# cvlab-stonybrook/s-volsdf

Measured on AMD Instinct MI355X. Metric: rendered rays/sec (1024-ray batch, 128 samples), higher is better.
Workload: dtype f32 (every product, forward and backward, as three fp16 MFMA products of two-piece fp16 operands with f32 accumulate; activation blocks hold both pieces: float32 accuracy class); 1 GPU; configs[1]: VolOpt.train_step (forward + MVS prior lookup + loss + backward + clip/guard/Adam), train mode, fast=1: 1024 rays/GPU x 128 coarse + 98 composited samples + 2048 eikonal points, 8x256 SDF MLP + 4x256 radiance MLP; mode=train, mlp_precision=fp16x2, launch=eager launches, rays_per_gpu=1024, rays_total=1024

## Files before the change

### s-volsdf_amd/csrc/svs_wgrad.hip

```cpp
#include "svs_common.h"
#include "svs_mlp_layout.h"
#include "svs_ticket.h"
#include <cstdlib>

namespace svs {
namespace wgrad {

struct Pair {
  const float* a;
  const float* b;
  size_t stride_a, stride_b;
};

struct Args {
  Pair p[2];
  int n_pairs;
  int n_tiles;
  int n_valid_points;
  const float* b_extra;
  size_t stride_extra;
  float* dW;
  int ldw;
  float* db;
  det::Ticket ticket;
};

struct Staging {
  f32x4 a[8], b[8], x;
};

template <int NTB>
__global__ __launch_bounds__(256, 1) void wgrad_kernel(Args a) {
  constexpr int PA = 260, PB = NTB == 9 ? 292 : 260;
  constexpr int BUF = 32 * (PA + PB);
  extern __shared__ __attribute__((aligned(16))) float smem[];
  const int tid = threadIdx.x, wave = tid >> 6, lane = tid & 63;
  const int half = lane >> 5, col = lane & 31;
  f32x16 acc[2][NTB];
#pragma unroll
  for (int o = 0; o < 2; ++o)
#pragma unroll
    for (int i = 0; i < NTB; ++i) acc[o][i] = (f32x16)(0.0f);
  float bias_acc = 0.0f;

  const int my_tiles = a.n_tiles > (int)blockIdx.x ? (a.n_tiles - 1 - (int)blockIdx.x) / (int)gridDim.x + 1 : 0;
  const int n_items = my_tiles * a.n_pairs;
  Staging st;
  int st_live = 32;

  auto issue = [&](int item) {
    const int t = blockIdx.x + (item / a.n_pairs) * gridDim.x, pi = item % a.n_pairs;
    const Pair& p = a.p[pi];
    const f32x4* ga = reinterpret_cast<const f32x4*>(p.a + (size_t)t * p.stride_a);
    const f32x4* gb = reinterpret_cast<const f32x4*>(p.b + (size_t)t * p.stride_b);
#pragma unroll
    for (int k = 0; k < 8; ++k) { st.a[k] = ga[k * 256 + tid]; st.b[k] = gb[k * 256 + tid]; }
    if (NTB == 9) {
      st.x = (a.b_extra && pi == 0) ? reinterpret_cast<const f32x4*>(a.b_extra + (size_t)t * a.stride_extra)[tid]
                                    : (f32x4)(0.0f);
    }
    st_live = a.n_valid_points - t * 32;
  };
  auto commit = [&](int buf) {
    float* la = smem + buf * BUF;
    float* lb = la + 32 * PA;
    if (st_live < 32) {
#pragma unroll
      for (int k = 0; k < 8; ++k) if ((tid & 31) >= st_live) st.a[k] = (f32x4)(0.0f);
    }
#pragma unroll
    for (int k = 0; k < 8; ++k) {
      const int q = k * 256 + tid, i4 = q >> 6, ln = q & 63;
      const int feat = 32 * (i4 >> 2) + 8 * (i4 & 3) + 4 * (ln >> 5), pt = ln & 31;
      *reinterpret_cast<f32x4*>(la + pt * PA + feat) = st.a[k];
      *reinterpret_cast<f32x4*>(lb + pt * PB + feat) = st.b[k];
    }
    if (NTB == 9) {
      const int i4 = tid >> 6, ln = tid & 63;
      *reinterpret_cast<f32x4*>(lb + (ln & 31) * PB + 256 + 8 * i4 + 4 * (ln >> 5)) = st.x;
    }
  };

  if (n_items > 0) { issue(0); commit(0); }
  __syncthreads();
  for (int item = 0; item < n_items; ++item) {
    const int buf = item & 1;
    const bool more = item + 1 < n_items;
    if (more) issue(item + 1);
    const float* la = smem + buf * BUF;
    const float* lb = la + 32 * PA;
    if (a.db && (item % a.n_pairs) == 0) {
      float s = 0.0f;
#pragma unroll 8
      for (int q = 0; q < 32; ++q) s += la[q * PA + tid];
      bias_acc += s;
    }
#pragma unroll 4
    for (int s = 0; s < 16; ++s) {
      const int pt = 2 * s + half;
      const float a0 = la[pt * PA + 32 * (2 * wave) + col];
      const float a1 = la[pt * PA + 32 * (2 * wave + 1) + col];
#pragma unroll
      for (int i = 0; i < NTB; ++i) {
        const float b = lb[pt * PB + 32 * i + col];
        acc[0][i] = __builtin_amdgcn_mfma_f32_32x32x2f32(a0, b, acc[0][i], 0, 0, 0);
        acc[1][i] = __builtin_amdgcn_mfma_f32_32x32x2f32(a1, b, acc[1][i], 0, 0, 0);
      }
    }
    if (more) commit(buf ^ 1);
    __syncthreads();
  }
  det::wait_turn(a.ticket, blockIdx.x);
#pragma unroll
  for (int o = 0; o < 2; ++o)
#pragma unroll
    for (int i = 0; i < NTB; ++i)
#pragma unroll
      for (int r = 0; r < 16; ++r) {
        const int row = 32 * (2 * wave + o) + rho(r) + 4 * half;
        const int c = 32 * i + col;
        if (c < a.ldw) atomicAdd(&a.dW[(size_t)row * a.ldw + c], acc[o][i][r]);
      }
  if (a.db) atomicAdd(&a.db[tid], bias_acc);
  det::pass_turn(a.ticket, blockIdx.x);
}


namespace h2 {

typedef _Float16 f16x8 __attribute__((ext_vector_type(8)));
typedef _Float16 f16x4 __attribute__((ext_vector_type(4)));
typedef _Float16 f16x2 __attribute__((ext_vector_type(2)));
typedef short s16x4 __attribute__((__vector_size__(4 * sizeof(short))));
#define SVS_LDS(T, ptr) ((__attribute__((address_space(3))) T*)(ptr))

constexpr int kPlane = 16384;
constexpr int kExtraPiece = 32 * 64;
constexpr int kNarrowImg = 8192;
constexpr int kRecBytes = 8 * 256;
constexpr int kFactorBytes = 8 * 64;
template <bool GP>
struct Ring {
  static constexpr int kPlanes = GP ? 2 : 1;
  static constexpr int kSlot = 2 * kPlanes * kPlane;
  static constexpr int kB = kPlanes * kPlane;
  static constexpr int kRing = GP ? 2 : 4;
  static constexpr int kAhead = kRing - 1;
  static constexpr int kSlotAll = kSlot + kRecBytes + kFactorBytes;
  static constexpr int kLdsBytes = kRing * kSlotAll;
};

struct Frag { s16x4 lo, hi; };
__device__ __forceinline__ void tr_issue(Frag& v, unsigned a0, unsigned a1) {
  asm volatile("ds_read_b64_tr_b16 %0, %1" : "=v"(v.lo) : "v"(a0));
  asm volatile("ds_read_b64_tr_b16 %0, %1" : "=v"(v.hi) : "v"(a1));
}
__device__ __forceinline__ f16x8 frag_of(const Frag& v) { return __builtin_bit_cast(f16x8, v); }
__device__ __forceinline__ void lds_read128(f32x4& v, unsigned a) { asm volatile("ds_read_b128 %0, %1" : "=v"(v) : "v"(a)); }
__device__ __forceinline__ void lds_read32(float& v, unsigned a) { asm volatile("ds_read_b32 %0, %1" : "=v"(v) : "v"(a)); }
__device__ __forceinline__ void lds_wait() {
  asm volatile("s_waitcnt lgkmcnt(0)" ::: "memory");
  __builtin_amdgcn_sched_barrier(0);
}
__device__ __forceinline__ unsigned lds_addr(const void* p) {
  return (unsigned)(unsigned long long)SVS_LDS(const void, p);
}

__device__ __forceinline__ void scale_from_absmax(const float* absmax, float& s, float& inv_s) {
  s = 1.0f; inv_s = 1.0f;
  if (!absmax) return;
  int e = (int)((__float_as_uint(*absmax) >> 23) & 0xff);
  e = e < 16 ? 16 : (e > 250 ? 250 : e);
  s = __uint_as_float((unsigned)(268 - e) << 23);
  inv_s = __uint_as_float((unsigned)(e - 14) << 23);
}

struct Job {
  Pair p[2];
  const float* rec[2];
  int n_pairs;
  int n_tiles;
  int n_valid_points;
  int b_tiles;
  int col0;
  float* dW;
  int ldw;
  float* db;
  const float* absmax;
  int wg_begin, wg_count;
  det::Ticket ticket;
};
constexpr int kMaxJobs = 20;
struct MultiArgs { Job job[kMaxJobs]; int n_jobs; int touch; int reverse; };
static_assert(sizeof(MultiArgs) <= 4096, "kernel arguments");

constexpr int kThreadsW = 512;

typedef const __attribute__((address_space(1))) void* gvoid;

template <bool GP>
__global__ __launch_bounds__(kThreadsW, 1) void wgrad_h2_multi_kernel(MultiArgs ma) {
  typedef Ring<GP> R;
  constexpr int kSlot = R::kSlot, kSlotAll = R::kSlotAll, kRing = R::kRing, kAhead = R::kAhead, kB = R::kB;
  extern __shared__ __attribute__((aligned(16))) unsigned char smem_h2[];
  int jj = 0;
  for (int q = 1; q < ma.n_jobs; ++q) if ((int)blockIdx.x >= ma.job[q].wg_begin) jj = q;
  const Job& a = ma.job[jj];
  const int wg = (int)blockIdx.x - a.wg_begin, nwg = a.wg_count;
  const int tid = threadIdx.x, lane = tid & 63;
  const int wave = __builtin_amdgcn_readfirstlane(tid >> 6);
  const bool narrow = a.b_tiles == 1;
  float s_grad, inv_s;
  scale_from_absmax(a.absmax, s_grad, inv_s);

  f32x16 acc[8];
#pragma unroll
  for (int i = 0; i < 8; ++i) acc[i] = (f32x16)(0.0f);
  float bsum = 0.0f;

  unsigned char* ring = smem_h2;

  const int rq = (lane & 15) >> 2, rp = lane & 3, rg = (lane >> 4) & 1, rh = lane >> 5;
  const int rd0 = 1024 * rg + 256 * rh + 128 * rg + 64 * (rp & 1) + 16 * rq + 8 * (rp >> 1);
  const int a_rd = 2048 * wave + rd0;
  const int rx0 = 64 * (8 * rh + rq) + 32 * rg + 8 * rp, rx1 = rx0 + 64 * 4;
  const int wp = lane & 31, whf = lane >> 5;
  const int wxoff = 64 * wp + 16 * (wave & 3) + 8 * whf;

  const bool two_pairs = a.n_pairs == 2;
  const int my_tiles = a.n_tiles > wg ? (a.n_tiles - 1 - wg) / nwg + 1 : 0;
  const int n_items = two_pairs ? 2 * my_tiles : my_tiles;
  const int n_valid = a.n_valid_points;
  const bool has_db = a.db != nullptr;
  const bool rev = ma.reverse != 0;
  const float* const pa0 = a.p[0].a; const float* const pb0 = a.p[0].b;
  const float* const pa1 = a.p[1].a; const float* const pb1 = a.p[1].b;
  const size_t sa0 = a.p[0].stride_a, sb0 = a.p[0].stride_b, sa1 = a.p[1].stride_a, sb1 = a.p[1].stride_b;
  const float* const rec0 = a.rec[0]; const float* const rec1 = a.rec[1];
  const bool has_scale = a.absmax != nullptr;
  auto tile_of = [&](int item) {
    const int k = two_pairs ? item >> 1 : item;
    return rev ? wg + (my_tiles - 1 - k) * nwg : wg + k * nwg;
  };

  auto issue = [&](int item) {
    const int t = tile_of(item), pi = two_pairs ? item & 1 : 0;
    const float* pa = (pi ? pa1 : pa0) + (size_t)t * (pi ? sa1 : sa0);
    const float* pb = (pi ? pb1 : pb0) + (size_t)t * (pi ? sb1 : sb0);
    unsigned char* slot = ring + (item % kRing) * kSlotAll;
#pragma unroll
    for (int j = 0; j < 2 * R::kPlanes; ++j) {
      const int piece = wave + 8 * j;
      __builtin_amdgcn_global_load_lds((gvoid)(reinterpret_cast<const f32x4*>(pa) + piece * 64 + lane),
                                       SVS_LDS(void, slot + piece * 1024), 16, 0, 0);
      if (!narrow)
        __builtin_amdgcn_global_load_lds((gvoid)(reinterpret_cast<const f32x4*>(pb) + piece * 64 + lane),
                                         SVS_LDS(void, slot + kB + piece * 1024), 16, 0, 0);
    }
    if (narrow)
      __builtin_amdgcn_global_load_lds((gvoid)(reinterpret_cast<const f32x4*>(pb) + (wave & 3) * 64 + lane),
                                       SVS_LDS(void, slot + kB + (wave & 3) * 1024), 16, 0, 0);
    if (has_scale)
      __builtin_amdgcn_global_load_lds((gvoid)((pi ? rec1 : rec0) + (size_t)t * 64 + lane),
                                       SVS_LDS(void, slot + kSlot + wave * 256), 4, 0, 0);
  };
  unsigned sink = 0;
  auto touch = [&](int item) {
    const int t = tile_of(item), pi = two_pairs ? item & 1 : 0;
    const Pair& p = a.p[pi];
    constexpr int kLines = R::kPlanes * (kPlane / 128);
    const int nb = narrow ? 32 : kLines;
    const float* q = tid < kLines ? p.a + (size_t)t * p.stride_a + tid * 32
                                  : p.b + (size_t)t * p.stride_b + (tid - kLines) * 32;
    if (tid < kLines + nb) asm volatile("global_load_dword %0, %1, off" : "+v"(sink) : "v"(q) : "memory");
  };
  const int ops = (narrow ? 2 * R::kPlanes + 1 : 4 * R::kPlanes) + (has_scale ? 1 : 0);

  auto stage_factors = [&](int item) {
    unsigned char* slot = ring + (item % kRing) * kSlotAll;
    const int t = tile_of(item);
    const int live = n_valid - t * 32;
    float f = 1.0f;
    if (has_scale) {
      float rec;
      lds_read32(rec, lds_addr(slot + kSlot + wave * 256 + 4 * wp));
      lds_wait();
      const unsigned eb = (__float_as_uint(rec) >> 23) & 0xff;
      if (eb >= 20 && eb <= 240) f = __builtin_fminf(s_grad * __uint_as_float((254u << 23) - __float_as_uint(rec)), 32768.0f);
    }
    if (wp >= live) f = 0.0f;
    if (lane < 32) asm volatile("ds_write_b16 %0, %1" :: "v"(lds_addr(slot + kSlot + kRecBytes + wave * 64 + 2 * lane)), "v"((_Float16)f) : "memory");
  };
  auto stage_narrow = [&](int item) {
    unsigned char* slot = ring + (item % kRing) * kSlotAll;
    if (tid < 256) {
      f32x4 v;
      lds_read128(v, lds_addr(slot + kB + tid * 16));
      lds_wait();
      f16x4 hi, mid;
#pragma unroll
      for (int j = 0; j < 4; ++j) {
        const _Float16 h = (_Float16)v[j];
        hi[j] = h;
        mid[j] = (_Float16)(v[j] - (float)h);
      }
      *SVS_LDS(f16x4, slot + kB + kNarrowImg + wxoff) = hi;
      *SVS_LDS(f16x4, slot + kB + kNarrowImg + kExtraPiece + wxoff) = mid;
    }
  };

  const f16x2 one2 = {(_Float16)1.0f, (_Float16)1.0f};

  for (int i0 = 0; i0 < kAhead && i0 < n_items; ++i0) issue(i0);
  const bool touching = GP && ma.touch;
  bool touched = false;
  if (touching && kAhead < n_items) { touch(kAhead); touched = true; }
  auto pre_stage = [&](int it) {
    const int left = n_items - 1 - it;
    const int later = (left < kAhead - 1 ? left : kAhead - 1) * ops;
    if (later == 10) asm volatile("s_waitcnt vmcnt(10)" ::: "memory");
    else if (later == 8) asm volatile("s_waitcnt vmcnt(8)" ::: "memory");
    else if (later == 6) asm volatile("s_waitcnt vmcnt(6)" ::: "memory");
    else if (later == 5) asm volatile("s_waitcnt vmcnt(5)" ::: "memory");
    else if (later == 4) asm volatile("s_waitcnt vmcnt(4)" ::: "memory");
    else if (later == 3) asm volatile("s_waitcnt vmcnt(3)" ::: "memory");
    else if (touched) asm volatile("s_waitcnt vmcnt(1)" ::: "memory");
    else asm volatile("s_waitcnt vmcnt(0)" ::: "memory");
    stage_factors(it);
  };
  for (int item = 0; item < n_items; ++item) {
    const int pi = two_pairs ? item & 1 : 0;
    const bool p0 = pi == 0;
    pre_stage(item);
    asm volatile("s_waitcnt lgkmcnt(0)\n\ts_barrier" ::: "memory");
    if (narrow) {
      stage_narrow(item);
      asm volatile("s_waitcnt lgkmcnt(0)\n\ts_barrier" ::: "memory");
    }
    auto issue_next = [&]() {
      if (item + kAhead < n_items) issue(item + kAhead);
      touched = false;
      if (touching && item + kAhead + 1 < n_items) { touch(item + kAhead + 1); touched = true; }
    };
    const unsigned la = lds_addr(ring + (item % kRing) * kSlotAll);
    const unsigned lb = la + kB;
    const unsigned ftab = la + kSlot + kRecBytes + wave * 64;
    const unsigned nimg = lb + kNarrowImg;
    const bool want_bias = has_db && p0;
    const bool two = narrow;
    Frag fa2[2], fam2[2];
    f32x4 fraw2[2];
#pragma unroll
    for (int ks = 0; ks < 2; ++ks) {
      tr_issue(fa2[ks], la + 512 * ks + a_rd, la + 512 * ks + (a_rd ^ 128));
      if (GP) tr_issue(fam2[ks], la + kPlane + 512 * ks + a_rd, la + kPlane + 512 * ks + (a_rd ^ 128));
      lds_read128(fraw2[ks], ftab + 32 * ks + 16 * rh);
    }
    issue_next();
    lds_wait();
#pragma unroll
    for (int ks = 0; ks < 2; ++ks) {
      const f16x8 ah = frag_of(fa2[ks]) * __builtin_bit_cast(f16x8, fraw2[ks]);
      const f16x8 am = GP ? frag_of(fam2[ks]) * __builtin_bit_cast(f16x8, fraw2[ks]) : ah;
      if (want_bias) {
#pragma unroll
        for (int j = 0; j < 4; ++j) {
          const f16x2 h2v = {ah[2 * j], ah[2 * j + 1]};
          bsum = __builtin_amdgcn_fdot2(h2v, one2, bsum, false);
          if (GP) {
            const f16x2 m2v = {am[2 * j], am[2 * j + 1]};
            bsum = __builtin_amdgcn_fdot2(m2v, one2, bsum, false);
          }
        }
      }
#pragma unroll
      for (int i = 0; i < 8; ++i) {
        if (i > 0 && narrow) break;
        Frag fh, fm;
        if (!narrow) {
          const unsigned rd = lb + 2048 * i + 512 * ks + rd0;
          tr_issue(fh, rd, rd ^ 128);
          if (GP) tr_issue(fm, rd + kPlane, (rd ^ 128) + kPlane);
        } else {
          tr_issue(fh, nimg + ks * 1024 + rx0, nimg + ks * 1024 + rx1);
          tr_issue(fm, nimg + kExtraPiece + ks * 1024 + rx0, nimg + kExtraPiece + ks * 1024 + rx1);
        }
        lds_wait();
        if (two || GP) acc[i] = __builtin_amdgcn_mfma_f32_32x32x16_f16(ah, frag_of(fm), acc[i], 0, 0, 0);
        if (GP) acc[i] = __builtin_amdgcn_mfma_f32_32x32x16_f16(am, frag_of(fh), acc[i], 0, 0, 0);
        acc[i] = __builtin_amdgcn_mfma_f32_32x32x16_f16(ah, frag_of(fh), acc[i], 0, 0, 0);
      }
    }
  }
  asm volatile("s_waitcnt vmcnt(0)" :: "v"(sink) : "memory");
  const int half = lane >> 5, col = lane & 31;
  det::wait_turn(a.ticket, wg);
#pragma unroll
  for (int i = 0; i < 8; ++i) {
    if (i > 0 && narrow) break;
#pragma unroll
    for (int r = 0; r < 16; ++r) {
      const int row = 32 * wave + rho(r) + 4 * half;
      const int c = a.col0 + 32 * i + col;
      if (c < a.ldw) atomicAdd(&a.dW[(size_t)row * a.ldw + c], acc[i][r] * inv_s);
    }
  }
  if (a.db) {
    bsum += __shfl_xor(bsum, 32);
    if (half == 0) atomicAdd(&a.db[32 * wave + col], bsum * inv_s);
  }
  det::pass_turn(a.ticket, wg);
}

}

}
}

using namespace svs;
using namespace svs::wgrad;
namespace h2 = svs::wgrad::h2;

extern "C" {

struct svs_wgrad_job {
  const float *a0, *b0; long long sa0, sb0;
  const float *a1, *b1; long long sa1, sb1;
  const float* b_extra; long long s_extra;
  int n_points, ldw;
  float *dW, *db;
  const float* absmax;
  const float *rec0, *rec1;
};

int svs_wgrad_multi(const svs_wgrad_job* jobs, int n_jobs, int precision, void* hip_stream) {
  if (!jobs || n_jobs < 1) { set_error("svs_wgrad_multi: no jobs"); return SVS_EINVAL; }
  int n_expanded = 0;
  for (int j = 0; j < n_jobs; ++j) n_expanded += jobs[j].b_extra ? 2 : 1;
  if (n_expanded > h2::kMaxJobs) { set_error("svs_wgrad_multi: at most %d jobs (b_extra counts twice)", h2::kMaxJobs); return SVS_EINVAL; }
  for (int j = 0; j < n_jobs; ++j) {
    const svs_wgrad_job& q = jobs[j];
    if (!q.a0 || !q.b0 || !q.dW || q.n_points <= 0 || q.ldw < 256 || q.ldw > 288 || (q.b_extra && q.ldw < 288) || (q.a1 && !q.b1)) {
      set_error("svs_wgrad_multi: bad argument in job %d", j); return SVS_EINVAL;
    }
    if (mlp::is_h2(precision) && q.absmax && (!q.rec0 || (q.a1 && !q.rec1))) {
      set_error("svs_wgrad_multi: job %d has absmax but no scale records", j); return SVS_EINVAL;
    }
  }
  hipStream_t s = (hipStream_t)hip_stream;
  if (mlp::is_h2(precision)) {
    const bool gp = precision == mlp::kFmtF16x2;
    h2::MultiArgs ma;
    int n = 0;
    long long work[h2::kMaxJobs], total = 0;
    for (int j = 0; j < n_jobs; ++j) {
      const svs_wgrad_job& q = jobs[j];
      h2::Job& J = ma.job[n];
      J.p[0] = Pair{q.a0, q.b0, (size_t)q.sa0, (size_t)q.sb0};
      J.rec[0] = q.rec0; J.rec[1] = q.rec1;
      J.n_pairs = 1;
      if (q.a1) { J.p[1] = Pair{q.a1, q.b1, (size_t)q.sa1, (size_t)q.sb1}; J.n_pairs = 2; }
      else { J.p[1] = J.p[0]; J.rec[1] = J.rec[0]; }
      J.n_tiles = (q.n_points + 31) / 32; J.n_valid_points = q.n_points;
      J.b_tiles = 8; J.col0 = 0; J.dW = q.dW; J.ldw = q.ldw; J.db = q.db; J.absmax = q.absmax;
      work[n] = (long long)J.n_tiles * J.n_pairs * 10;
      total += work[n++];
      if (q.b_extra) {
        h2::Job& X = ma.job[n];
        X = J;
        X.p[0].b = q.b_extra; X.p[0].stride_b = (size_t)q.s_extra; X.n_pairs = 1;
        X.b_tiles = 1; X.col0 = 256; X.db = nullptr;
        work[n] = (long long)X.n_tiles * 6;
        total += work[n++];
      }
    }
    ma.n_jobs = n;
    static const int touch_env = [] { const char* e = getenv("SVS_WGRAD_TOUCH"); return e ? atoi(e) : 0; }();
    ma.touch = touch_env;
    static const int reverse_env = [] { const char* e = getenv("SVS_WGRAD_REVERSE"); return e ? atoi(e) : 0; }();
    ma.reverse = reverse_env;
    (void)total;
    const int n_wg_total = 256;
    int count[h2::kMaxJobs];
    int used = 0;
    for (int j = 0; j < n; ++j) { count[j] = 1; ++used; }
    while (used < n_wg_total) {
      int best = -1;
      double load = 0.0;
      for (int j = 0; j < n; ++j) {
        if (count[j] >= ma.job[j].n_tiles) continue;
        const double l = (double)work[j] / count[j];
        if (l > load) { load = l; best = j; }
      }
      if (best < 0) break;
      ++count[best]; ++used;
    }
    int begin = 0;
    for (int j = 0; j < n; ++j) {
      ma.job[j].wg_begin = begin; ma.job[j].wg_count = count[j];
      begin += count[j];
      ma.job[j].ticket = det::Ticket{nullptr, 0u, 0u};
    }
    if (deterministic()) {
      int owner[h2::kMaxJobs], n_owner = 0;
      for (int j = 0; j < n; ++j) {
        owner[j] = -1;
        for (int k = 0; k < j; ++k)
          if (ma.job[k].dW == ma.job[j].dW && ma.job[k].col0 == ma.job[j].col0) { owner[j] = owner[k]; break; }
        if (owner[j] < 0) owner[j] = n_owner++;
      }
      unsigned* turn = det::take_slots((unsigned)n_owner);
      if (!turn) { set_error("svs_wgrad_multi: no turn counters (deterministic mode)"); return SVS_EINVAL; }
      unsigned total[h2::kMaxJobs] = {0};
      for (int j = 0; j < n; ++j) { ma.job[j].ticket.turn = turn + owner[j]; ma.job[j].ticket.first = total[owner[j]]; total[owner[j]] += (unsigned)count[j]; }
      for (int j = 0; j < n; ++j) ma.job[j].ticket.total = total[owner[j]];
    }
    static hipError_t e = hipFuncSetAttribute(reinterpret_cast<const void*>(h2::wgrad_h2_multi_kernel<false>),
                                              hipFuncAttributeMaxDynamicSharedMemorySize, h2::Ring<false>::kLdsBytes);
    static hipError_t ep = hipFuncSetAttribute(reinterpret_cast<const void*>(h2::wgrad_h2_multi_kernel<true>),
                                               hipFuncAttributeMaxDynamicSharedMemorySize, h2::Ring<true>::kLdsBytes);
    if (e != hipSuccess || ep != hipSuccess) {
      set_error("svs_wgrad_multi: hipFuncSetAttribute: %s", hipGetErrorString(e != hipSuccess ? e : ep)); return (int)(e != hipSuccess ? e : ep);
    }
    if (gp) h2::wgrad_h2_multi_kernel<true><<<begin, h2::kThreadsW, h2::Ring<true>::kLdsBytes, s>>>(ma);
    else h2::wgrad_h2_multi_kernel<false><<<begin, h2::kThreadsW, h2::Ring<false>::kLdsBytes, s>>>(ma);
    return check_launch("svs_wgrad_multi");
  }
  if (precision != mlp::kFmtF32) { set_error("svs_wgrad_multi: unknown precision %d", precision); return SVS_EINVAL; }
  for (int j = 0; j < n_jobs; ++j) {
    const svs_wgrad_job& q = jobs[j];
    Args a;
    a.p[0] = Pair{q.a0, q.b0, (size_t)q.sa0, (size_t)q.sb0};
    a.n_pairs = 1;
    if (q.a1) { a.p[1] = Pair{q.a1, q.b1, (size_t)q.sa1, (size_t)q.sb1}; a.n_pairs = 2; }
    a.n_tiles = (q.n_points + 31) / 32;
    a.n_valid_points = q.n_points;
    a.b_extra = q.b_extra; a.stride_extra = (size_t)q.s_extra;
    a.dW = q.dW; a.ldw = q.ldw; a.db = q.db;
    const int grid = a.n_tiles < 256 ? a.n_tiles : 256;
    a.ticket = det::Ticket{det::take_slots(1), 0u, (unsigned)grid};
    if (q.b_extra) {
      constexpr int lds = 2 * 32 * (260 + 292) * 4;
      static hipError_t e9 = hipFuncSetAttribute(reinterpret_cast<const void*>(wgrad_kernel<9>),
                                                 hipFuncAttributeMaxDynamicSharedMemorySize, lds);
      if (e9 != hipSuccess) { set_error("svs_wgrad_multi: hipFuncSetAttribute: %s", hipGetErrorString(e9)); return (int)e9; }
      wgrad_kernel<9><<<grid, 256, lds, s>>>(a);
    } else {
      constexpr int lds = 2 * 32 * (260 + 260) * 4;
      static hipError_t e8 = hipFuncSetAttribute(reinterpret_cast<const void*>(wgrad_kernel<8>),
                                                 hipFuncAttributeMaxDynamicSharedMemorySize, lds);
      if (e8 != hipSuccess) { set_error("svs_wgrad_multi: hipFuncSetAttribute: %s", hipGetErrorString(e8)); return (int)e8; }
      wgrad_kernel<8><<<grid, 256, lds, s>>>(a);
    }
    if (int rc = check_launch("svs_wgrad_multi")) return rc;
  }
  return SVS_OK;
}

int svs_wgrad(const float* a0, const float* b0, long long sa0, long long sb0, const float* a1, const float* b1,
              long long sa1, long long sb1, const float* b_extra, long long s_extra, int n_points, int precision,
              const float* absmax, const float* rec0, const float* rec1, float* dW, int ldw, float* db, void* hip_stream) {
  svs_wgrad_job q{a0, b0, sa0, sb0, a1, b1, sa1, sb1, b_extra, s_extra, n_points, ldw, dW, db, absmax, rec0, rec1};
  return svs_wgrad_multi(&q, 1, precision, hip_stream);
}

}
```

Measured before the change: 298,200 rays/s.

## Switch wgrad MFMA to 16x16x32 tiles with conflict-free LDS read maps

Replaces the 32x32x16 MFMA tiling in the weight-gradient kernel with 16x16x32 MFMAs over a 2x16 accumulator grid per wave. The K dimension of 32 points per tile is now consumed in one instruction instead of two k-steps. LDS transposed-read address maps are rebuilt, with compile-time checks for bank conflicts, and use immediate offsets. The factor table and narrow B image layout are permuted to match. This changes operand reuse and register pressure, and the write-back becomes more atomics of smaller fragments.

```diff
diff --git a/s-volsdf_amd/csrc/svs_wgrad.hip b/s-volsdf_amd/csrc/svs_wgrad.hip
--- a/s-volsdf_amd/csrc/svs_wgrad.hip
+++ b/s-volsdf_amd/csrc/svs_wgrad.hip
@@ -1,7 +1,9 @@
 #include "svs_common.h"
 #include "svs_mlp_layout.h"
 #include "svs_ticket.h"
+#include "svs_wgrad_maps.h"
 #include <cstdlib>
+#include <type_traits>
 
 namespace svs {
 namespace wgrad {
@@ -151,9 +153,18 @@
 };
 
 struct Frag { s16x4 lo, hi; };
-__device__ __forceinline__ void tr_issue(Frag& v, unsigned a0, unsigned a1) {
-  asm volatile("ds_read_b64_tr_b16 %0, %1" : "=v"(v.lo) : "v"(a0));
-  asm volatile("ds_read_b64_tr_b16 %0, %1" : "=v"(v.hi) : "v"(a1));
+template <int OFF>
+__device__ __forceinline__ void tr_issue(Frag& v, unsigned base) {
+  static_assert(OFF >= 0 && OFF + 256 < 65536, "ds offset field");
+  asm volatile("ds_read_b64_tr_b16 %0, %1 offset:%2" : "=v"(v.lo) : "v"(base), "n"(OFF));
+  asm volatile("ds_read_b64_tr_b16 %0, %1 offset:%2" : "=v"(v.hi) : "v"(base), "n"(OFF + 256));
+}
+template <int N, typename F>
+__device__ __forceinline__ void static_for(F&& f) {
+  if constexpr (N > 0) {
+    static_for<N - 1>(f);
+    f(std::integral_constant<int, N - 1>{});
+  }
 }
 __device__ __forceinline__ f16x8 frag_of(const Frag& v) { return __builtin_bit_cast(f16x8, v); }
 __device__ __forceinline__ void lds_read128(f32x4& v, unsigned a) { asm volatile("ds_read_b128 %0, %1" : "=v"(v) : "v"(a)); }
@@ -195,6 +206,11 @@
 static_assert(sizeof(MultiArgs) <= 4096, "kernel arguments");
 
 constexpr int kThreadsW = 512;
+constexpr int kRT = 2, kCT = 16;
+static_assert(maps::plane_reads_ok(kPlane), "transposed reads of the operand planes: bank conflict");
+static_assert(maps::narrow_reads_ok(kExtraPiece), "transposed reads of the narrow B image: bank conflict");
+static_assert(kPlane % 256 == 0 && kNarrowImg % 256 == 0 && kExtraPiece % 256 == 0 && Ring<true>::kSlotAll % 256 == 0 &&
+              Ring<false>::kSlotAll % 256 == 0, "every region the reads are offset by starts on a 256-byte bank row");
 
 typedef const __attribute__((address_space(1))) void* gvoid;
 
@@ -213,19 +229,24 @@
   float s_grad, inv_s;
   scale_from_absmax(a.absmax, s_grad, inv_s);
 
-  f32x16 acc[8];
-#pragma unroll
-  for (int i = 0; i < 8; ++i) acc[i] = (f32x16)(0.0f);
-  float bsum = 0.0f;
+  f32x4 acc[kRT][kCT];
+#pragma unroll
+  for (int o = 0; o < kRT; ++o)
+#pragma unroll
+    for (int i = 0; i < kCT; ++i) acc[o][i] = (f32x4)(0.0f);
+  float bsum[kRT];
+#pragma unroll
+  for (int o = 0; o < kRT; ++o) bsum[o] = 0.0f;
 
   unsigned char* ring = smem_h2;
 
-  const int rq = (lane & 15) >> 2, rp = lane & 3, rg = (lane >> 4) & 1, rh = lane >> 5;
-  const int rd0 = 1024 * rg + 256 * rh + 128 * rg + 64 * (rp & 1) + 16 * rq + 8 * (rp >> 1);
-  const int a_rd = 2048 * wave + rd0;
-  const int rx0 = 64 * (8 * rh + rq) + 32 * rg + 8 * rp, rx1 = rx0 + 64 * 4;
+  const int rg = lane >> 4;
+  const int rd_even = maps::plane_base(0, lane), rd_odd = maps::plane_base(1, lane);
+  const int a_off = 1024 * kRT * wave;
+  const int rx = maps::narrow_base(lane);
   const int wp = lane & 31, whf = lane >> 5;
-  const int wxoff = 64 * wp + 16 * (wave & 3) + 8 * whf;
+  const int wxoff = maps::narrow_at(8 * (wave & 3) + 4 * whf, wp);
+  const int n_ct = narrow ? 2 : kCT;
 
   const bool two_pairs = a.n_pairs == 2;
   const int my_tiles = a.n_tiles > wg ? (a.n_tiles - 1 - wg) / nwg + 1 : 0;
@@ -289,7 +310,7 @@
       if (eb >= 20 && eb <= 240) f = __builtin_fminf(s_grad * __uint_as_float((254u << 23) - __float_as_uint(rec)), 32768.0f);
     }
     if (wp >= live) f = 0.0f;
-    if (lane < 32) asm volatile("ds_write_b16 %0, %1" :: "v"(lds_addr(slot + kSlot + kRecBytes + wave * 64 + 2 * lane)), "v"((_Float16)f) : "memory");
+    if (lane < 32) asm volatile("ds_write_b16 %0, %1" :: "v"(lds_addr(slot + kSlot + kRecBytes + wave * 64 + 2 * maps::factor_pos(wp))), "v"((_Float16)f) : "memory");
   };
   auto stage_narrow = [&](int item) {
     unsigned char* slot = ring + (item % kRing) * kSlotAll;
@@ -345,69 +366,86 @@
     const unsigned la = lds_addr(ring + (item % kRing) * kSlotAll);
     const unsigned lb = la + kB;
     const unsigned ftab = la + kSlot + kRecBytes + wave * 64;
-    const unsigned nimg = lb + kNarrowImg;
+    const unsigned a_even = la + a_off + rd_even, a_odd = la + a_off + rd_odd;
+    const unsigned b_even = lb + rd_even, b_odd = lb + rd_odd;
+    const unsigned n_rd = lb + kNarrowImg + rx;
     const bool want_bias = has_db && p0;
     const bool two = narrow;
-    Frag fa2[2], fam2[2];
-    f32x4 fraw2[2];
-#pragma unroll
-    for (int ks = 0; ks < 2; ++ks) {
-      tr_issue(fa2[ks], la + 512 * ks + a_rd, la + 512 * ks + (a_rd ^ 128));
-      if (GP) tr_issue(fam2[ks], la + kPlane + 512 * ks + a_rd, la + kPlane + 512 * ks + (a_rd ^ 128));
-      lds_read128(fraw2[ks], ftab + 32 * ks + 16 * rh);
-    }
+    Frag fa[kRT], fam[kRT];
+    f32x4 fraw;
+    static_for<kRT>([&](auto oc) {
+      constexpr int o = decltype(oc)::value;
+      tr_issue<1024 * o>(fa[o], o & 1 ? a_odd : a_even);
+      if (GP) tr_issue<kPlane + 1024 * o>(fam[o], o & 1 ? a_odd : a_even);
+    });
+    lds_read128(fraw, ftab + 16 * rg);
     issue_next();
     lds_wait();
-#pragma unroll
-    for (int ks = 0; ks < 2; ++ks) {
-      const f16x8 ah = frag_of(fa2[ks]) * __builtin_bit_cast(f16x8, fraw2[ks]);
-      const f16x8 am = GP ? frag_of(fam2[ks]) * __builtin_bit_cast(f16x8, fraw2[ks]) : ah;
+    f16x8 ah[kRT], am[kRT];
+#pragma unroll
+    for (int o = 0; o < kRT; ++o) {
+      ah[o] = frag_of(fa[o]) * __builtin_bit_cast(f16x8, fraw);
+      am[o] = GP ? frag_of(fam[o]) * __builtin_bit_cast(f16x8, fraw) : ah[o];
       if (want_bias) {
 #pragma unroll
         for (int j = 0; j < 4; ++j) {
-          const f16x2 h2v = {ah[2 * j], ah[2 * j + 1]};
-          bsum = __builtin_amdgcn_fdot2(h2v, one2, bsum, false);
+          const f16x2 h2v = {ah[o][2 * j], ah[o][2 * j + 1]};
+          bsum[o] = __builtin_amdgcn_fdot2(h2v, one2, bsum[o], false);
           if (GP) {
-            const f16x2 m2v = {am[2 * j], am[2 * j + 1]};
-            bsum = __builtin_amdgcn_fdot2(m2v, one2, bsum, false);
+            const f16x2 m2v = {am[o][2 * j], am[o][2 * j + 1]};
+            bsum[o] = __builtin_amdgcn_fdot2(m2v, one2, bsum[o], false);
           }
         }
       }
-#pragma unroll
-      for (int i = 0; i < 8; ++i) {
-        if (i > 0 && narrow) break;
+    }
+    static_for<kCT>([&](auto ic) {
+      constexpr int i = decltype(ic)::value;
+      if (i < n_ct) {
         Frag fh, fm;
         if (!narrow) {
-          const unsigned rd = lb + 2048 * i + 512 * ks + rd0;
-          tr_issue(fh, rd, rd ^ 128);
-          if (GP) tr_issue(fm, rd + kPlane, (rd ^ 128) + kPlane);
-        } else {
-          tr_issue(fh, nimg + ks * 1024 + rx0, nimg + ks * 1024 + rx1);
-          tr_issue(fm, nimg + kExtraPiece + ks * 1024 + rx0, nimg + kExtraPiece + ks * 1024 + rx1);
+          tr_issue<1024 * i>(fh, i & 1 ? b_odd : b_even);
+          if (GP) tr_issue<kPlane + 1024 * i>(fm, i & 1 ? b_odd : b_even);
+        } else if constexpr (i < 2) {
+          tr_issue<1024 * i>(fh, n_rd);
+          tr_issue<kExtraPiece + 1024 * i>(fm, n_rd);
         }
         lds_wait();
-        if (two || GP) acc[i] = __builtin_amdgcn_mfma_f32_32x32x16_f16(ah, frag_of(fm), acc[i], 0, 0, 0);
-        if (GP) acc[i] = __builtin_amdgcn_mfma_f32_32x32x16_f16(am, frag_of(fh), acc[i], 0, 0, 0);
-        acc[i] = __builtin_amdgcn_mfma_f32_32x32x16_f16(ah, frag_of(fh), acc[i], 0, 0, 0);
-      }
-    }
+        const f16x8 bh = frag_of(fh), bm = frag_of(fm);
+        if (two || GP) {
+#pragma unroll
+          for (int o = 0; o < kRT; ++o) acc[o][i] = __builtin_amdgcn_mfma_f32_16x16x32_f16(ah[o], bm, acc[o][i], 0, 0, 0);
+        }
+        if (GP) {
+#pragma unroll
+          for (int o = 0; o < kRT; ++o) acc[o][i] = __builtin_amdgcn_mfma_f32_16x16x32_f16(am[o], bh, acc[o][i], 0, 0, 0);
+        }
+#pragma unroll
+        for (int o = 0; o < kRT; ++o) acc[o][i] = __builtin_amdgcn_mfma_f32_16x16x32_f16(ah[o], bh, acc[o][i], 0, 0, 0);
+      }
+    });
   }
   asm volatile("s_waitcnt vmcnt(0)" :: "v"(sink) : "memory");
-  const int half = lane >> 5, col = lane & 31;
+  const int fcol = lane & 15;
   det::wait_turn(a.ticket, wg);
-#pragma unroll
-  for (int i = 0; i < 8; ++i) {
-    if (i > 0 && narrow) break;
-#pragma unroll
-    for (int r = 0; r < 16; ++r) {
-      const int row = 32 * wave + rho(r) + 4 * half;
-      const int c = a.col0 + 32 * i + col;
-      if (c < a.ldw) atomicAdd(&a.dW[(size_t)row * a.ldw + c], acc[i][r] * inv_s);
-    }
-  }
+  static_for<kCT>([&](auto ic) {
+    constexpr int i = decltype(ic)::value;
+    const int c = a.col0 + 16 * i + fcol;
+    if (i < n_ct && c < a.ldw) {
+#pragma unroll
+      for (int o = 0; o < kRT; ++o)
+#pragma unroll
+        for (int r = 0; r < 4; ++r)
+          atomicAdd(&a.dW[(size_t)(16 * (kRT * wave + o) + 4 * rg + r) * a.ldw + c], acc[o][i][r] * inv_s);
+    }
+  });
   if (a.db) {
-    bsum += __shfl_xor(bsum, 32);
-    if (half == 0) atomicAdd(&a.db[32 * wave + col], bsum * inv_s);
+#pragma unroll
+    for (int o = 0; o < kRT; ++o) {
+      float sum = bsum[o];
+      sum += __shfl_xor(sum, 16);
+      sum += __shfl_xor(sum, 32);
+      if (lane < 16) atomicAdd(&a.db[16 * (kRT * wave + o) + lane], sum * inv_s);
+    }
   }
   det::pass_turn(a.ticket, wg);
 }
diff --git a/s-volsdf_amd/csrc/svs_wgrad_maps.h b/s-volsdf_amd/csrc/svs_wgrad_maps.h
--- /dev/null
+++ b/s-volsdf_amd/csrc/svs_wgrad_maps.h
@@ -0,0 +1,96 @@
+#pragma once
+
+namespace svs {
+namespace wgrad {
+namespace h2 {
+namespace maps {
+
+constexpr int quad_of(int g, int r) { return 4 * (g >> 1) + (g & 1) + 2 * r; }
+
+constexpr int point_of(int g, int j) { return 4 * quad_of(g, j >> 2) + (j & 3); }
+
+constexpr int plane_rd(int s, int lane, int r) {
+  const int g = lane >> 4, q = (lane & 15) >> 2, p = lane & 3, a = quad_of(g, r);
+  return 1024 * s + 256 * (a >> 1) + 128 * ((a & 1) ^ (s & 1)) + 64 * (p & 1) + 16 * q + 8 * (p >> 1);
+}
+constexpr int plane_base(int parity, int lane) { return plane_rd(parity, lane, 0) - 1024 * parity; }
+
+constexpr int narrow_at(int feature, int point) { return 1024 * (feature >> 4) + 32 * point + 2 * (feature & 15); }
+constexpr int narrow_rd(int c, int lane, int r) {
+  const int g = lane >> 4, q = (lane & 15) >> 2, p = lane & 3;
+  return narrow_at(16 * c + 4 * p, 4 * quad_of(g, r) + q);
+}
+constexpr int narrow_base(int lane) { return narrow_rd(0, lane, 0); }
+
+constexpr int factor_pos(int point) {
+  const int a = point >> 2;
+  return 8 * (2 * (a >> 2) + (a & 1)) + 4 * ((a >> 1) & 1) + (point & 3);
+}
+
+constexpr bool half_rows_ok(const int (&addr)[64]) {
+  for (int h = 0; h < 2; ++h) {
+    bool seen[32] = {};
+    const int row = addr[32 * h] >> 8;
+    for (int l = 0; l < 32; ++l) {
+      const int b = addr[32 * h + l];
+      if ((b & 7) || (b >> 8) != row) return false;
+      const int slot = (b & 255) >> 3;
+      if (seen[slot]) return false;
+      seen[slot] = true;
+    }
+  }
+  return true;
+}
+
+constexpr bool plane_reads_ok(int plane_bytes) {
+  for (int plane = 0; plane < 2; ++plane)
+    for (int s = 0; s < 16; ++s)
+      for (int r = 0; r < 2; ++r) {
+        int addr[64] = {};
+        for (int l = 0; l < 64; ++l) {
+          addr[l] = plane * plane_bytes + plane_rd(s, l, r);
+          if (plane_rd(s, l, r) != plane_base(s & 1, l) + 1024 * s + 256 * r) return false;
+        }
+        if (!half_rows_ok(addr)) return false;
+      }
+  return true;
+}
+constexpr bool narrow_reads_ok(int piece_bytes) {
+  for (int piece = 0; piece < 2; ++piece)
+    for (int c = 0; c < 2; ++c)
+      for (int r = 0; r < 2; ++r) {
+        int addr[64] = {};
+        for (int l = 0; l < 64; ++l) {
+          addr[l] = piece * piece_bytes + narrow_rd(c, l, r);
+          if (narrow_rd(c, l, r) != narrow_base(l) + 1024 * c + 256 * r) return false;
+        }
+        if (!half_rows_ok(addr)) return false;
+      }
+  return true;
+}
+constexpr bool factor_table_ok() {
+  bool seen[32] = {};
+  for (int g = 0; g < 4; ++g)
+    for (int j = 0; j < 8; ++j) {
+      const int pt = point_of(g, j);
+      if (pt < 0 || pt >= 32 || seen[pt] || factor_pos(pt) != 8 * g + j) return false;
+      seen[pt] = true;
+    }
+  return true;
+}
+constexpr bool natural_order_conflicts() {
+  int addr[64] = {};
+  for (int l = 0; l < 64; ++l) {
+    const int g = l >> 4, q = (l & 15) >> 2, p = l & 3, a = 2 * g;
+    addr[l] = 256 * (a >> 1) + 128 * (a & 1) + 64 * (p & 1) + 16 * q + 8 * (p >> 1);
+  }
+  return !half_rows_ok(addr);
+}
+
+static_assert(factor_table_ok(), "factor table does not follow the fragments' point order");
+static_assert(natural_order_conflicts(), "the conflict check accepts a map known to conflict");
+
+}
+}
+}
+}
```

Measured after the change: 302,600 rays/s, median of 6. +1.5%, better.
